# balaji1312/cassnat_asr_public

Measured on AMD Instinct MI355X. Metric: utterances_per_sec, higher is better.
Workload: dtype bf16; 1 GPU; BASELINE configs[1]: CASS-NAT 12L-enc / 1+3+2 dec blocks, d_model 256, 4 heads, d_ff 2048, V 5000, greedy NAST; 32 utterances x 1000 frames x 80 fbank per GPU per step; batch_per_gpu=32, frames=1000, feat_dim=80, global_batch=32, parallelism=utterance-sharded x1, decode_pipelines_per_gpu=2, batches_per_engine_pass=10, utterances_per_engine_pass=320, row_predictions=208, row_predictions_missed=0

## Files before the change

cassnat_asr_public_amd/csrc/conv2.hip:

```cpp
#include <algorithm>
#include <cmath>
#include <cstdlib>
#include <cstring>

#include "kernels.h"

struct Conv2Params {
    const unsigned char* A;
    const unsigned char* W;
    const unsigned char* A_lo;
    const unsigned char* W_lo;
    const int* q8;
    const unsigned char* A8l;
    const unsigned char* A8q;
    const unsigned char* W8q;
    const unsigned char* W8l;
    float out8_scale;
    const float* bias;
    bf16* out;
    int M, T1, F1, T2, F2, ntiles;
    long long lda_bytes;
    int ksteps;
    float* out_f32;
    const float* pe;
    int pe_period;
    float scale;
};

constexpr int C2_BM = 256, C2_N = 256, C2_C = 256, C2_ROWB = 128;
constexpr int C2_SLAB = C2_BM * C2_ROWB;
constexpr int C2_WBASE = 3 * C2_SLAB;
constexpr int C2_OSTRIDE = 528;
constexpr int C2_LDS = 5 * C2_SLAB;
static_assert(C2_BM * C2_OSTRIDE <= C2_LDS && C2_BM == C2_N, "epilogue image fits; A and W slabs are the same size");
static_assert(C2_LDS <= 160 * 1024, "LDS budget");
constexpr int C2_KSTEPS = 9 * (C2_C / 64);
constexpr int C2_LIN8_KSTEPS = 40;

#define C2_STR2(x) #x
#define C2_STR(x) C2_STR2(x)
#define C2_MF CN_MFMA16_ASM
#define C2_DMA(src, dst)                                                                              \
    __builtin_amdgcn_global_load_lds((const __attribute__((address_space(1))) void*)(src),          \
                                     (__attribute__((address_space(3))) void*)(dst), 16, 0, 0)
#ifdef C2_EXP_NO_READ
#define C2_RDA(i) ""
#define C2_RDW(i) ""
#else
#define C2_RDA(i) "ds_read_b128 %[na" #i "], %[an] offset:" C2_STR(i * 4096) "\n\t"
// ... 43 lines not shown
#define C2_BLOCK8(PRE, A0c, W0c, A1c, W1c, A0n, W0n, A1n, W1n, DMA, vo)                                        \
    asm volatile(PRE "s_waitcnt lgkmcnt(0)\n\t"                                                                \
                 C2_M8(0, 0) C2_RDA8(0) C2_M8(0, 1) C2_RDA8(1) C2_M8(0, 2) C2_RDA8(2) C2_M8(0, 3) C2_RDA8(3)   \
                 C2_M8(1, 0) C2_RDW8(0) C2_M8(1, 1) C2_RDW8(1) C2_M8(1, 2) C2_RDW8(2) C2_M8(1, 3) C2_RDW8(3)   \
                 C2_M8(2, 0) DMA(0) C2_M8(2, 1) DMA(1) C2_M8(2, 2) DMA(2) C2_M8(2, 3) DMA(3)                   \
                 C2_M8(3, 0) DMA(4) C2_M8(3, 1) DMA(5) C2_M8(3, 2) DMA(6) C2_M8(3, 3) DMA(7)                   \
                 : [c00] "+a"(acc[0]), [c01] "+a"(acc[1]), [c02] "+a"(acc[2]), [c03] "+a"(acc[3]), [c10] "+a"(acc[4]), \
                   [c11] "+a"(acc[5]), [c12] "+a"(acc[6]), [c13] "+a"(acc[7]), [c20] "+a"(acc[8]), [c21] "+a"(acc[9]), \
                   [c22] "+a"(acc[10]), [c23] "+a"(acc[11]), [c30] "+a"(acc[12]), [c31] "+a"(acc[13]),          \
                   [c32] "+a"(acc[14]), [c33] "+a"(acc[15]), [na0] "=&v"(A0n[0]), [na1] "=&v"(A0n[1]),          \
                   [na2] "=&v"(A0n[2]), [na3] "=&v"(A0n[3]), [nb0] "=&v"(A1n[0]), [nb1] "=&v"(A1n[1]),          \
                   [nb2] "=&v"(A1n[2]), [nb3] "=&v"(A1n[3]), [nw0] "=&v"(W0n[0]), [nw1] "=&v"(W0n[1]),          \
                   [nw2] "=&v"(W0n[2]), [nw3] "=&v"(W0n[3]), [nv0] "=&v"(W1n[0]), [nv1] "=&v"(W1n[1]),          \
                   [nv2] "=&v"(W1n[2]), [nv3] "=&v"(W1n[3]), [tv] "+v"(tv_)                                    \
                 : [a0] "v"(C2_JOIN(A0c[0], A1c[0])), [a1] "v"(C2_JOIN(A0c[1], A1c[1])), [a2] "v"(C2_JOIN(A0c[2], A1c[2])), \
                   [a3] "v"(C2_JOIN(A0c[3], A1c[3])), [w0] "v"(C2_JOIN(W0c[0], W1c[0])), [w1] "v"(C2_JOIN(W0c[1], W1c[1])), \
                   [w2] "v"(C2_JOIN(W0c[2], W1c[2])), [w3] "v"(C2_JOIN(W0c[3], W1c[3])), [an0] "v"(an0_), [an1] "v"(an1_), \
                   [wn0] "v"(wn0_), [wn1] "v"(wn1_), [vo0] "v"(vo[0]), [vo1] "v"(vo[1]), [vo2] "v"(vo[2]), [vo3] "v"(vo[3]), \
                   [vo4] "v"(vo[4]), [vo5] "v"(vo[5]), [vo6] "v"(vo[6]), [vo7] "v"(vo[7]), [st] "s"(st_), [sb] "s"(sb_), \
                   [qa] "v"(qa_), [qb] "v"(qb_), [wstep] "s"(wstep_)                                           \
                 : "memory", "scc")
typedef int c2_v4i __attribute__((ext_vector_type(4)));

template <bool LINEAR, bool X3 = false, bool F8 = false, bool MIX = false>
__global__ __launch_bounds__(256) void conv2_kernel(Conv2Params p) {
    static_assert(!(LINEAR && X3) && !(F8 && X3), "the split form exists for the convolution only; e4m3: convolution and linear_out");
    static_assert(!MIX || (!LINEAR && !X3 && !F8), "MIX is a form of the convolution of its own");
    constexpr int ES = F8 ? 1 : 2;
    extern __shared__ __attribute__((aligned(16))) unsigned char smem[];
    const int tid = threadIdx.x, lane = tid & 63;
    const int wave = __builtin_amdgcn_readfirstlane(tid >> 6);
    const int wm = wave >> 1, wnn = wave & 1;
    const int half = lane >> 5, l31 = lane & 31;
    const int nwg = gridDim.x, xcd = blockIdx.x & 7, q = nwg >> 3, rm = nwg & 7;
    const int tile = (xcd < rm ? xcd * (q + 1) : rm * (q + 1) + (xcd - rm) * q) + (blockIdx.x >> 3);
    const int m0 = tile * C2_BM;

    const int r8 = lane >> 3, cp = lane & 7;
    const unsigned sw = (unsigned)((cp ^ ((4 * wave + (r8 >> 1)) & 7)) << 4);
    const int F1p = p.F1 + 2;
    auto a_off = [&](int mm, int es) -> long long {
        if constexpr (LINEAR) return (long long)mm * p.lda_bytes;
        const int f2 = mm % p.F2, bt = mm / p.F2;
        const int t2 = bt % p.T2, b = bt / p.T2;
        return (((long long)b * (p.T1 + 2) + 2 * t2) * F1p + 2 * f2) * (C2_C * es);
    };
    long long tile_off = a_off(m0, ES);
    unsigned pa[8], pw[8];
#pragma unroll
    for (int i = 0; i < 8; ++i) {
        const int row = 8 * (wave + 4 * i) + r8;
        const int m = m0 + row;
        const int mc = m < p.M ? m : p.M - 1;
        pa[i] = (unsigned)(a_off(mc, ES) - tile_off) + sw;
        if constexpr (LINEAR)
            pw[i] = (unsigned)(row * (p.ksteps * 128)) + sw;
        else
            pw[i] = (unsigned)(row * (9 * C2_C * ES)) + sw;
// ... 332 lines not shown
            for (int g = 0; g < 4; ++g) bv[g] = *reinterpret_cast<const f32x4*>(p.bias + wnn * 128 + 32 * nt + 8 * g + 4 * half);
#pragma unroll
            for (int mt = 0; mt < 4; ++mt)
#pragma unroll
                for (int g = 0; g < 4; ++g) {
                    bf16x4 o;
#pragma unroll
                    for (int e = 0; e < 4; ++e) o[e] = (bf16)fmaxf(acc[4 * nt + mt][4 * g + e] + bv[g][e], 0.f);
                    *reinterpret_cast<bf16x4*>(orow + mt * 32 * C2_OSTRIDE + (32 * nt + 8 * g) * 2) = o;
                }
        }
    }
    __syncthreads();
#pragma unroll
    for (int it = 0; it < 32; ++it) {
        const int row = 8 * it + (tid >> 5), ch = tid & 31;
        const int m = m0 + row;
        if (m < p.M)
            *reinterpret_cast<uint4*>(reinterpret_cast<unsigned char*>(p.out) + (long long)m * 512 + ch * 16) =
                *reinterpret_cast<const uint4*>(smem + row * C2_OSTRIDE + ch * 16);
    }
}

bool conv2_dma_applies(int prec, int C, int N) { return prec == CN_PREC_BF16 && C == C2_C && N == C2_N && !cn_exp_env("CASSNAT_NO_CONV2_DMA"); }

static bool conv2_tile_span_too_large(int T1, int F1, int F2) {
    const long long span = ((256ll / (F2 > 0 ? F2 : 1) + 3) * 2 + 4) * (F1 + 2) * C2_C * 2;
    if (span >= (1ll << 32)) {
        cn_set_error("conv2: one 256-row tile spans more than 4 GiB of the image (feature dimension too wide for the LDS-DMA kernel)");
        return true;
    }
    (void)T1;
    return false;
}

int launch_conv2_dma(const void* in, const void* w, const float* bias, void* out, int B, int T1, int F1, int T2, int F2,
                     hipStream_t s) {
    static CnAttrOnce attr_once;
    int attr_dev;
    if (attr_once.need(&attr_dev)) {
        CN_HIP_CHECK(hipFuncSetAttribute((const void*)conv2_kernel<false>, hipFuncAttributeMaxDynamicSharedMemorySize, C2_LDS));
        attr_once.mark(attr_dev);
    }
    Conv2Params p;
    p.A = (const unsigned char*)in;
    p.W = (const unsigned char*)w;
// ... 123 lines not shown
    p.A8l = p.A + 2 * cells;
    p.A8q = p.A + 3 * cells;
    p.W = (const unsigned char*)w_hi;
    p.W8q = (const unsigned char*)w8q;
    p.W8l = (const unsigned char*)w8l;
    p.q8 = q8_dev;
    p.bias = bias;
    p.out = (bf16*)out;
    p.M = B * T2 * F2;
    p.T1 = T1;
    p.F1 = F1;
    p.T2 = T2;
    p.F2 = F2;
    p.ntiles = cn_ceil_div(p.M, C2_BM);
    if (p.M <= 0) return 0;
    hipLaunchKernelGGL((conv2_kernel<false, false, false, true>), dim3(p.ntiles), dim3(256), C2_LDS, s, p);
    CN_HIP_CHECK(hipGetLastError());
    return 0;
}

bool linear256_dma_applies(int prec, int N, int K) { return prec == CN_PREC_BF16 && N == C2_N && K % 64 == 0 && K >= 128 && !cn_exp_env("CASSNAT_NO_LINEAR_DMA"); }

int launch_linear256_dma(const void* A, int lda, const void* W, const float* bias, float* out, int M, int K, float scale,
                         const float* pe, int pe_period, hipStream_t s) {
    static CnAttrOnce attr_once;
    int attr_dev;
    if (attr_once.need(&attr_dev)) {
        CN_HIP_CHECK(hipFuncSetAttribute((const void*)conv2_kernel<true>, hipFuncAttributeMaxDynamicSharedMemorySize, C2_LDS));
        attr_once.mark(attr_dev);
    }
    if (M <= 0) return 0;
    if (256ll * lda * 2 >= (1ll << 32)) {
        cn_set_error("linear256: a 256-row tile of A exceeds the 32-bit lane offsets of the LDS-DMA kernel");
        return -1;
    }
    Conv2Params p = {};
    p.A = (const unsigned char*)A;
    p.W = (const unsigned char*)W;
    p.bias = bias;
    p.M = M;
    p.T1 = p.F1 = p.T2 = p.F2 = 1;
    p.ntiles = cn_ceil_div(M, C2_BM);
    p.lda_bytes = (long long)lda * 2;
    p.ksteps = K / 64;
    p.out_f32 = out;
    p.pe = pe;
    p.pe_period = pe_period > 0 ? pe_period : 1;
    p.scale = scale;
    hipLaunchKernelGGL(conv2_kernel<true>, dim3(p.ntiles), dim3(256), C2_LDS, s, p);
    CN_HIP_CHECK(hipGetLastError());
    return 0;
}

template <typename F>
static void c2_each_weight(const float* w, int C, long long s_co, long long s_tap, long long s_ci, F f) {
    size_t e = 0;
    for (int co = 0; co < C; ++co)
        for (int tap = 0; tap < 9; ++tap)
            for (int ci = 0; ci < C; ++ci) f(e++, w[co * s_co + tap * s_tap + ci * s_ci]);
}
static int c2_e4m3_exp(const float* w, int C, long long s_co, long long s_tap, long long s_ci) {
    float mx = 0.f;
    c2_each_weight(w, C, s_co, s_tap, s_ci, [&](size_t, float v) { mx = std::max(mx, std::fabs(v)); });
    return cn_e4m3_exp(mx);
}

int pack_conv2_f8(const float* w, int C, long long s_co, long long s_tap, long long s_ci, unsigned char* out) {
    const int lg = c2_e4m3_exp(w, C, s_co, s_tap, s_ci);
    const float scale = std::ldexp(1.f, lg);
    c2_each_weight(w, C, s_co, s_tap, s_ci, [&](size_t e, float v) { out[e] = cn_f32_to_e4m3_host(v * scale); });
    return lg;
// ... 16 lines not shown
```

cassnat_asr_public_amd/csrc/gemm.hip:

```cpp
#include "kernels.h"

struct GemmParams {
    const unsigned char* A;
    const unsigned char* W;
    const float* bias;
    void* C;
    const float* resid;
    const float* pe;
    long long lda_bytes;
    int ldc, ldr;
    int M, N, K;
    int epi;
    int pe_period;
    float scale, resid_scale;
    const float* w_inv_scale;
    float acc_scale, c_scale;
    int ntn;
    int cT1, cF1, cC, cT2, cF2;
};

template <typename T, typename TC, int BM, int BN, bool CONV, bool FULLK = false>
__global__ __launch_bounds__(256) void gemm_kernel(GemmParams p) {
    constexpr int ROWB = 128;
    constexpr int BK = ROWB / (int)sizeof(T);
// ... 280 lines not shown

static int dispatch_gemm_fp8(const GemmArgs& a, hipStream_t s) {
    if (a.M <= 0 || a.N <= 0) return 0;
    if (a.conv || a.K <= 0 || a.K % 128 != 0 || a.lda % 16 != 0) {
        cn_set_error("gemm(fp8): K must be a positive multiple of 128 and rows 16-byte aligned; no convolution form");
        return -1;
    }
    const bool use_big = (long long)cn_ceil_div(a.M, 128) * cn_ceil_div(a.N, 128) >= 512;
    if (a.c_f32) return use_big ? run_gemm<fp8_t, float, 128, 128, false>(a, s) : run_gemm<fp8_t, float, 64, 64, false>(a, s);
    if (a.c_fp8) return use_big ? run_gemm<fp8_t, fp8_t, 128, 128, false>(a, s) : run_gemm<fp8_t, fp8_t, 64, 64, false>(a, s);
    return use_big ? run_gemm<fp8_t, bf16, 128, 128, false>(a, s) : run_gemm<fp8_t, bf16, 64, 64, false>(a, s);
}

int launch_gemm(int prec, const GemmArgs& a, hipStream_t s) {
    if (a.ab_fp8) return dispatch_gemm_fp8(a, s);
    if (a.conv && a.conv_halo) {
        if (!(a.epi == CN_EPI_RELU && a.ldc == a.N && conv2_dma_applies(prec, a.cC, a.N))) {
            cn_set_error("gemm: a haloed conv input is only understood by the bf16 256-channel conv2 kernel");
            return -1;
        }
        return launch_conv2_dma(a.A, a.W, a.bias, a.C, a.cB, a.cT1, a.cF1, a.cT2, a.cF2, s);
    }
    if (!a.conv && a.epi == CN_EPI_EMBED && a.c_f32 && a.ldc == a.N && a.K >= 1024 && linear256_dma_applies(prec, a.N, a.K))
        return launch_linear256_dma(a.A, a.lda, a.W, a.bias, (float*)a.C, a.M, a.K, a.scale, a.pe, a.pe_period, s);
    if (prec == CN_PREC_X3) {
        if (a.lda % 32 != 0 || (!a.c_f32 && a.ldc % 32 != 0)) {
            cn_set_error("gemm: split-bf16 operands need row strides that are multiples of 32 elements");
            return -1;
        }
        return dispatch_gemm<split_t>(a, s);
    }
    return prec == CN_PREC_F32 ? dispatch_gemm<float>(a, s) : dispatch_gemm<bf16>(a, s);
}
```

cassnat_asr_public_amd/csrc/kernels.h:

```cpp
#pragma once
#include "common.h"

enum { CN_PREC_F32 = 0, CN_PREC_BF16 = 1, CN_PREC_X3 = 3 };
static inline size_t cn_elem_size(int prec) { return prec == CN_PREC_BF16 ? 2 : 4; }

enum { CN_EPI_RELU = 1, CN_EPI_RESID = 2, CN_EPI_EMBED = 4, CN_EPI_SWISH = 8 };
struct GemmArgs {
    const void* A = nullptr;
    int lda = 0;
    const void* W = nullptr;
    const float* bias = nullptr;
    void* C = nullptr;
    int ldc = 0;
    int c_f32 = 0;
    int M = 0, N = 0, K = 0;
    int epi = 0;
    const float* resid = nullptr;
    float resid_scale = 1.0f;
    int ldr = 0;
    const float* pe = nullptr;
    int pe_period = 1;
    float scale = 1.f;
    int ab_fp8 = 0;
    float acc_scale = 1.f;
    const float* w_inv_scale = nullptr;
    int c_fp8 = 0;
    float c_scale = 1.f;
    int conv = 0;
    int conv_halo = 0;
    int cB = 0, cT1 = 0, cF1 = 0, cC = 0, cT2 = 0, cF2 = 0;
};
int launch_gemm(int prec, const GemmArgs& a, hipStream_t s);

struct UttMeta {
    int frames;
    int tp;
    int sub_lo;
    int sub_hi;
};
int launch_conv1(int prec, const float* x, const float* w9c, const float* bias, void* out, int B, int T, int F, int T1,
                 int F1, int C, int halo, hipStream_t s, const UttMeta* utt_meta = nullptr);
int launch_conv1_planes(const float* x, const float* w9c, const float* bias, void* out, int B, int T, int F, int T1, int F1,
                        int C, int halo, hipStream_t s, const UttMeta* utt_meta = nullptr);
int launch_conv1_mixplanes(const float* x, const float* w9c, const float* bias, void* out, int B, int T, int F, int T1, int F1, int C,
                           int halo, float scale_l, float scale_q, hipStream_t s, const UttMeta* utt_meta = nullptr);
int launch_conv1_f8(const float* x, const float* w9c, const float* bias, void* out8, int B, int T, int F, int T1, int F1, int C,
                    int halo, float scale, hipStream_t s, const UttMeta* utt_meta = nullptr);
bool conv1_bordered_bf16_applies(int C, int F1);
int launch_conv1_bordered_bf16(const float* x, const float* w9c, const float* bias, void* out, int B, int T, int F, int T1, int F1,
                               int C, hipStream_t s, const UttMeta* utt_meta = nullptr);
constexpr int CN_MAX_SUB = 64;
struct SubList {
    int n;
// ... 190 lines not shown
                   long long capacity);
int launch_wave_resample(int in_rate, int out_rate, const unsigned char* staged, long long staged_bytes, const int* off, const int* samples,
                         const int* channels, const int* channel, int utts, const int* rows, int n_rows, long long max_out, float* out,
                         const int* out_off, hipStream_t s);

bool conv2_dma_applies(int prec, int C, int N);
bool conv2_f8_applies(int C, int N);
int launch_conv2_f8(const void* in8, const void* w8, const int* q8_dev, const float* bias, void* out, int B, int T1, int F1, int T2,
                    int F2, hipStream_t s, float out8_scale = 0.f);
bool linear256_f8_applies(int N, int K);
int launch_linear256_f8(const void* A8, const void* W8, const int* q8_dev, const float* bias, float* out, int M, int K, float scale,
                        const float* pe, int pe_period, hipStream_t s);
bool conv2_mix_applies(int prec, int C, int N);
int launch_conv2_mix(const void* img, const void* w_hi, const void* w8q, const void* w8l, const int* q8_dev, const float* bias, void* out,
                     int B, int T1, int F1, int T2, int F2, hipStream_t s);
constexpr int MIX_LG_AQ = 0, MIX_LG_AL = 11;
int pack_conv2_f8(const float* w, int C, long long s_co, long long s_tap, long long s_ci, unsigned char* out);
void pack_conv2_mix(const float* w, int C, long long s_co, long long s_tap, long long s_ci, unsigned char* out, int* q8);
bool conv2_x3_applies(int prec, int C, int N);
int launch_conv2_x3(const void* in_hi, const void* in_lo, const void* w_hi, const void* w_lo, const float* bias, void* out, int B,
                    int T1, int F1, int T2, int F2, hipStream_t s);
bool linear256_dma_applies(int prec, int N, int K);
int launch_linear256_dma(const void* A, int lda, const void* W, const float* bias, float* out, int M, int K, float scale,
                         const float* pe, int pe_period, hipStream_t s);
int launch_conv2_dma(const void* in, const void* w, const float* bias, void* out, int B, int T1, int F1, int T2, int F2,
                     hipStream_t s);

constexpr int CHAIN_TAB_FLOATS = 5120;
constexpr int CHAIN_UNIT_BYTES = 16384;
struct ChainArgs {
    float* x = nullptr;
    const void* ctx = nullptr;
    int ldctx = 0;
    int ctx_blocked = 0;
    const void* wstream = nullptr;
    const float* tab = nullptr;
    void* out = nullptr;
    int ldo = 0;
    void* ln_out = nullptr;
    int ld_ln = 0;
    int M = 0, d = 0, dff = 0, tail_n = 0, has_next = 0;
    const int* m_dev = nullptr;
    int x_in_blocked = 0, x_out_blocked = 0, store_x = 1;
    int out_blocked = 0;
    int swish = 0;
    int f8 = 0;
    const int* f8_q = nullptr;
// ... 199 lines not shown
```

cassnat_asr_public_amd/csrc/model.hip:

```cpp
#include <algorithm>
#include <cmath>
#include <cstring>
#include <map>
#include <memory>
#include <string>
#include <thread>
#include <vector>

#include "../../include/cassnat_hip.h"
#include "kernels.h"

static thread_local std::string g_last_error;
static const int g_lib_tag = 0;
void cn_set_error(const std::string& msg) { g_last_error = msg; }
extern "C" const char* cn_last_error(void) { return g_last_error.c_str(); }
extern "C" const char* cn_version(void) { return "cassnat_hip 0.1 (gfx950, 16-bit operand " CN_OP16_NAME ")"; }
extern "C" const char* cn_operand16(void) { return CN_OP16_NAME; }

int cn_own_precision(int32_t precision, const char* who) {
#ifdef CN_OP16_F16
    if (precision == CN_PRECISION_F16) return CN_PREC_BF16;
    cn_set_error(std::string(who) + ": this build of the library (libcassnat_hip_f16.so) holds the fp16 engine only (CN_PRECISION_F16)");
    return -1;
#else
// ... 1858 lines not shown
        if (mix_planes) {
            const size_t wn = (size_t)d * 9 * d;
            const unsigned char* w = (const unsigned char*)m->conv2_mixw;
            CN_TRY(launch_conv2_mix(m->c1, w, w + 2 * wn, w + 3 * wn, m->conv2_mixq, m->conv2.b, m->c2, B, T1, F1, Tp, F2, s));
        } else if (x3_planes) {
            const size_t img = (size_t)B * (T1 + 2) * (F1 + 2) * d * 2, wpl = (size_t)d * 9 * d * 2;
            CN_TRY(launch_conv2_x3(m->c1, (const unsigned char*)m->c1 + img, m->conv2_x3w, (const unsigned char*)m->conv2_x3w + wpl,
                                   m->conv2.b, m->c2, B, T1, F1, Tp, F2, s));
        } else if (f8_img) {
            CN_TRY(launch_conv2_f8(m->c1, m->conv2_f8w, m->conv2_f8q, m->conv2.b, m->c2, B, T1, F1, Tp, F2, s, f8_lin ? FP8_S_IMG : 0.f));
        } else {
            CN_TRY(launch_gemm(m->prec, g, s));
        }
    }
    if (cap && !f8_lin) CN_TRY(capture(m, "conv2", m->c2, true, CN_DTYPE_F32, {B, Tp, F2, d}, s));
    if (f8_lin) {
        ProfScope ps(m, "linear_out_embed", 2.0 * M * d * (double)F2 * d, (double)M * F2 * d + (double)d * F2 * d + (double)M * d * 4, s);
        CN_TRY(launch_linear256_f8(m->c2, m->linear_f8w, m->linear_f8q, m->linear_out.b, m->x, M, F2 * d, sqrtf((float)d),
                                   c.conf_enc ? nullptr : m->pe, Tp, s));
    } else {
        GemmArgs g;
        g.A = m->c2;
        g.lda = F2 * d;
        g.W = m->linear_out.W;
        g.bias = m->linear_out.b;
        g.C = m->x;
        g.ldc = d;
        g.c_f32 = 1;
        g.M = M;
        g.N = d;
        g.K = F2 * d;
        g.epi = CN_EPI_EMBED;
        g.pe = c.conf_enc ? nullptr : m->pe;
        g.pe_period = Tp;
        g.scale = sqrtf((float)d);
        ProfScope ps(m, "linear_out_embed", 2.0 * g.M * g.N * g.K,
                     ((double)g.M * g.K + (double)g.N * g.K) * m->es + (double)g.M * g.N * 4, s);
        CN_TRY(launch_gemm(m->prec, g, s));
    }
    if (cap) CN_TRY(capture(m, "x_embed", m->x, false, CN_DTYPE_F32, {B, Tp, d}, s));
    static const bool no_chain_c = cn_exp_env("CASSNAT_NO_CHAIN") != nullptr;
    if (c.conf_enc && !m->enc.empty() && m->enc[0].cf_a.w && !no_chain_c) {
        for (size_t n = 0; n < m->enc.size(); ++n) {
            const bool last = n + 1 == m->enc.size();
            const int xin = (cap || n == 0) ? 0 : CHX_IN_BLK, xout = cap ? 0 : (last ? CHX_NO_STORE : CHX_OUT_BLK);
            CN_TRY(run_conformer_layer_chain(m, m->enc[n], m->x, B, Tp, m->keymask, nullptr, false, 0, nullptr, cap, xin, xout,
                                             last ? m->enc_h : nullptr, s));
            if (cap) CN_TRY(capture(m, ("enc_layer" + std::to_string(n)).c_str(), m->x, false, CN_DTYPE_F32, {B, Tp, d}, s));
        }
        if (cap) CN_TRY(capture(m, "enc_h", m->enc_h, true, CN_DTYPE_F32, {B, Tp, d}, s));
        return 0;
    }
    if (c.conf_enc) {
        for (size_t n = 0; n < m->enc.size(); ++n) {
            CN_TRY(run_conformer_self_layer(m, m->enc[n], m->x, B, Tp, m->keymask, nullptr, s));
            if (cap) CN_TRY(capture(m, ("enc_layer" + std::to_string(n)).c_str(), m->x, false, CN_DTYPE_F32, {B, Tp, d}, s));
        }
        CN_TRY(run_ln(m, m->enc_norm, m->x, m->enc_h, M, s));
        if (cap) CN_TRY(capture(m, "enc_h", m->enc_h, true, CN_DTYPE_F32, {B, Tp, d}, s));
        return 0;
    }
    static const bool no_chain = cn_exp_env("CASSNAT_NO_CHAIN") != nullptr;
    if (m->fp8_enc && (m->enc_chain.size() != m->enc.size() || no_chain)) {
// ... 1899 lines not shown
```

cassnat_asr_public_amd/csrc/ops.hip:

```cpp
#include <algorithm>
#include <cmath>
#include <cstring>
#include <string>
#include <thread>
#include <vector>

#include "../../include/cassnat_hip.h"
#include "kernels.h"

namespace {

class Scratch {
  public:
    Scratch(const char* who, hipStream_t s) : who_(who), s_(s) {}
    Scratch(const Scratch&) = delete;
    Scratch& operator=(const Scratch&) = delete;
    ~Scratch() {
        (void)hipStreamSynchronize(s_);
        for (void* p : bufs_) (void)hipFree(p);
    }
    bool ok() const { return ok_; }
    void* alloc(size_t bytes) {
        if (!ok_) return nullptr;
        void* p = nullptr;
// ... 306 lines not shown
    g.N = C;
    g.K = 9 * C;
    g.epi = CN_EPI_RELU;
    g.conv = 1;
    g.cB = B;
    g.cT1 = T1;
    g.cF1 = F1;
    g.cC = C;
    g.cT2 = T2;
    g.cF2 = F2;
    if (!conv2_dma_applies(precision, C, C)) return launch_gemm(precision, g, (hipStream_t)stream);
    const size_t cell = (size_t)C * 2, prow = (size_t)(F1 + 2) * cell;
    Scratch sc("cn_op_conv2", (hipStream_t)stream);
    void* padded = sc.alloc((size_t)B * (T1 + 2) * prow);
    if (!sc.ok()) return -2;
    CN_HIP_CHECK(hipMemsetAsync(padded, 0, (size_t)B * (T1 + 2) * prow, (hipStream_t)stream));
    for (int b = 0; b < B; ++b)
        CN_HIP_CHECK(hipMemcpy2DAsync((unsigned char*)padded + ((size_t)b * (T1 + 2) + 1) * prow + cell, prow,
                                      (const unsigned char*)conv1_out + (size_t)b * T1 * F1 * cell, (size_t)F1 * cell,
                                      (size_t)F1 * cell, T1, hipMemcpyDeviceToDevice, (hipStream_t)stream));
    g.A = padded;
    g.conv_halo = 1;
    return sc.finish(launch_gemm(precision, g, (hipStream_t)stream));
}

extern "C" int cn_op_layernorm(int32_t precision, const float* x, const float* a2, const float* b2, void* y, int32_t M,
                               int32_t d, float eps, void* stream) {
    if ((precision = cn_own_precision(precision, "cn_op_layernorm")) < 0) return -1;
    return launch_layernorm(precision, x, a2, b2, y, 0, M, d, eps, (hipStream_t)stream);
}

static int conv_module_dims(const char* who, int precision, long long rows, long long row_len, int d, const char* what) {
    if (precision != CN_PREC_F32 && precision != CN_PREC_BF16 && precision != CN_PREC_X3) {
        cn_set_error(std::string(who) + ": precision must be F32, BF16 (F16 in the half-precision build) or BF16X3");
        return -1;
    }
    if (precision == CN_PREC_X3 && d % 32 != 0) {
        cn_set_error(std::string(who) + ": split-bf16 (bf16x3) rows are groups of 32 elements: d % 32 != 0 has no layout");
        return -1;
    }
    if (row_len * d > 0x7fffffffLL || rows * row_len > 0x7fffffffLL || rows * row_len * d >= (1LL << 39)) {
        cn_set_error(std::string(who) + ": " + what + " exceeds the kernels' int arithmetic (2^31 - 1; all elements together: 2^39)");
        return -1;
    }
    return 0;
}
// ... 1033 lines not shown
```

cassnat_asr_public_amd/hip.py:

```python
import ctypes as C
import os
import re

import numpy as np

_HERE = os.path.dirname(os.path.abspath(__file__))
LIB_PATH = os.environ.get("CASSNAT_HIP_LIB") or os.path.join(_HERE, "libcassnat_hip.so")
LIB_PATH_F16 = os.path.join(_HERE, "libcassnat_hip_f16.so")
HEADER_PATH = os.path.join(os.path.dirname(_HERE), "include", "cassnat_hip.h")

PRECISION = {"fp32": 0, "f32": 0, "float32": 0, "bf16": 1, "bfloat16": 1, "fp8": 2, "bf16x3": 3, "fp16": 4, "float16": 4}
DTYPES = {0: np.float32, 1: np.int32, 2: np.uint8, 3: np.float64}
FP8_SCOPE_BITS = {"conv2": 1, "linear": 2, "ffn": 4}


def parse_fp8_scope(text):
    text = (text or "all").strip().lower()
    if text == "all":
        return 0, 0
    scope, first = 0, 0
    for part in text.split("+"):
        name, _, arg = part.strip().partition(":")
        if name not in FP8_SCOPE_BITS or (arg and name != "ffn"):
            raise ValueError(f"hip_fp8_scope: unknown part {part!r} (all, or conv2 / linear / ffn[:first layer] joined by +)")
# ... 71 lines not shown
def lib(flavour=None):
    path = LIB_PATH_F16 if flavour == "f16" else LIB_PATH
    if path in _libs:
        return _libs[path]
    if not os.path.exists(path):
        raise HipError(f"{path} is missing: run `python -c 'import __graft_entry__ as g; g.build()'` "
                       "(there is no CPU fallback for the CASS-NAT hot path)")
    L = C.CDLL(path)
    L.cn_last_error.restype = C.c_char_p
    L.cn_version.restype = C.c_char_p
    L.cn_operand16.restype = C.c_char_p
    L.cn_model_destroy.restype = None
    for name in declared_symbols():
        fn = getattr(L, name)
        if name not in ("cn_last_error", "cn_version", "cn_operand16", "cn_model_destroy"):
            fn.restype = C.c_int
    L.cn_op_gemm.argtypes = [C.c_int32, C.c_void_p, C.c_int32, C.c_void_p, C.c_void_p, C.c_void_p, C.c_int32, C.c_int32,
                             C.c_int32, C.c_int32, C.c_int32, C.c_int32, C.c_void_p, C.c_int32, C.c_void_p, C.c_int32,
                             C.c_float, C.c_void_p]
    L.cn_op_convert.argtypes = [C.c_int32, C.c_void_p, C.c_void_p, C.c_int64, C.c_int32, C.c_void_p]
    L.cn_op_conv1.argtypes = [C.c_int32] + [C.c_void_p] * 4 + [C.c_int32] * 4 + [C.c_void_p]
    L.cn_op_conv1_bordered.argtypes = [C.c_void_p] * 4 + [C.c_int32] * 4 + [C.c_void_p]
    L.cn_op_conv2.argtypes = [C.c_int32] + [C.c_void_p] * 4 + [C.c_int32] * 4 + [C.c_void_p]
    L.cn_op_conv_frontend_fp8.argtypes = [C.c_void_p] * 7 + [C.c_int32] * 4 + [C.c_float, C.c_float, C.c_void_p, C.c_void_p]
    L.cn_op_conv_frontend_mix.argtypes = [C.c_void_p] * 7 + [C.c_int32] * 4 + [C.c_void_p]
    L.cn_op_linear256_fp8.argtypes = [C.c_void_p] * 4 + [C.c_int32] * 2 + [C.c_float, C.c_float, C.c_void_p, C.c_int32, C.c_void_p, C.c_void_p]
    L.cn_op_layernorm.argtypes = [C.c_int32] + [C.c_void_p] * 4 + [C.c_int32, C.c_int32, C.c_float, C.c_void_p]
    L.cn_op_glu.argtypes = [C.c_int32, C.c_void_p, C.c_void_p, C.c_int32, C.c_int32, C.c_void_p]
    L.cn_op_dwconv.argtypes = [C.c_int32] + [C.c_void_p] * 4 + [C.c_int32] * 5 + [C.c_void_p]
    L.cn_op_groupnorm_swish.argtypes = [C.c_int32] + [C.c_void_p] * 5 + [C.c_int32] * 3 + [C.c_float, C.c_void_p]
    L.cn_op_attention.argtypes = [C.c_int32, C.c_void_p, C.c_int32, C.c_void_p, C.c_int32, C.c_void_p, C.c_int32,
                                  C.c_void_p, C.c_int32, C.c_int32, C.c_int32, C.c_int32, C.c_int32, C.c_void_p,
                                  C.c_void_p, C.c_void_p, C.c_int32, C.c_int32, C.c_float, C.c_void_p]
    L.cn_op_attention_desc.argtypes = [C.c_int32, C.POINTER(CnAttnDesc), C.c_void_p]
    L.cn_attn_desc_size.argtypes = []
    L.cn_op_attention_packed.argtypes = [C.c_int32, C.POINTER(CnAttnDesc), C.c_void_p, C.c_int32, C.c_void_p]
    L.cn_op_row_plan.argtypes = [C.c_void_p, C.c_int32, C.c_int32, C.c_int32, C.c_int32, C.c_void_p, C.c_void_p, C.c_void_p, C.c_void_p]
    L.cn_op_logsoftmax_argmax.argtypes = [C.c_void_p, C.c_int32, C.c_int32, C.c_void_p, C.c_void_p, C.c_int32, C.c_void_p]
    L.cn_op_ctc_align.argtypes = [C.c_void_p] * 3 + [C.c_int32] * 5 + [C.c_void_p] * 6
    L.cn_op_greedy_pack.argtypes = [C.c_void_p] * 3 + [C.c_int32] * 4 + [C.c_void_p] * 4
    L.cn_op_ctc_prefix_beam.argtypes = [C.c_void_p, C.c_void_p, C.c_int32, C.c_int32, C.c_int32, C.c_int32, C.c_int32, C.c_double,
                                        C.c_int32, C.c_void_p, C.c_int32, C.c_void_p, C.c_void_p, C.c_void_p, C.c_void_p, C.c_void_p,
                                        C.c_void_p]
    L.cn_op_ctc_viterbi.argtypes = [C.c_void_p] * 5 + [C.c_int32] * 6 + [C.c_void_p, C.c_void_p]
    L.cn_op_topk.argtypes = [C.c_void_p, C.c_int32, C.c_int32, C.c_int32, C.c_void_p, C.c_void_p, C.c_void_p]
    L.cn_op_gemm_fp8.argtypes = [C.c_void_p, C.c_int32, C.c_void_p, C.c_void_p, C.c_void_p, C.c_int32, C.c_int32, C.c_int32, C.c_float,
# ... 289 lines not shown
            self._chk(self.L.cn_model_load_weights(self.handle, name.encode(), a.ctypes.data_as(C.c_void_p), shape, a.ndim),
                  f"load {name}")
        pe = np.ascontiguousarray(pe_table.detach().cpu().numpy() if hasattr(pe_table, "detach") else pe_table,
                                  dtype=np.float32)
        self._chk(self.L.cn_model_load_pe(self.handle, pe.ctypes.data_as(C.c_void_p), pe.shape[0]), "load pe")
        self.finalize()

    def finalize(self):
        self._chk(self.L.cn_model_finalize(self.handle), "cn_model_finalize")
        self.finalized = True

    def weight_blob(self):
        p, n = C.c_void_p(), C.c_int64()
        self._chk(self.L.cn_model_weight_blob(self.handle, C.byref(p), C.byref(n)), "cn_model_weight_blob")
        return p.value, n.value

    @staticmethod
    def make_opts(args, capture=False):
        opts = CnDecodeOpts(padding_idx=int(args.padding_idx), sos=1, left_trigger=int(getattr(args, "left_trigger", 0)),
                            right_trigger=int(getattr(args, "right_trigger", 0)), src_trigger=int(bool(getattr(args, "src_trigger", False))),
                            use_unimask=int(bool(getattr(args, "use_unimask", False))), beam_width=int(args.beam_width),
                            capture=int(bool(capture)), no_trigger=int(not getattr(args, "use_trigger", True)))
        opts.reserved[1] = int(bool(getattr(args, "hip_padded_rows", False)))
        return opts

    def decode(self, feats, size_ratio, opts, hyp, hyp_len, score):
        B, T, F = feats.shape
        self._chk(self.L.cn_decode_nast(self.handle, _ptr(feats), _ptr(size_ratio), B, T, F, C.byref(opts), _ptr(hyp),
                                    hyp.shape[1], _ptr(hyp_len), _ptr(score), current_stream()), "cn_decode_nast")

    def decode_merged(self, feats, size_ratio, opts, sub_rows, sub_frames, hyp, hyp_len, score, u_hint=0):
        B, T, F = feats.shape
        n = len(sub_rows) if sub_rows is not None else 0
        rows = (C.c_int32 * max(1, n))(*[int(x) for x in (sub_rows or [])])
        frames = (C.c_int32 * max(1, n))(*[int(x) for x in (sub_frames or [])])
        ticket = C.c_int32(-1)
        self._chk(self.L.cn_decode_nast_merged(self.handle, _ptr(feats), _ptr(size_ratio), B, T, F, C.byref(opts), n, rows, frames,
                                           int(u_hint), _ptr(hyp), hyp.shape[1], _ptr(hyp_len), _ptr(score), current_stream(),
                                           C.byref(ticket)), "cn_decode_nast_merged")
        return ticket.value

    def check_range(self, what="decode"):
        if self.precision not in ("fp16", "float16", "bf16x3"):
            return
        fault, limit = C.c_int32(), C.c_float()
        self._chk(self.L.cn_take_range_fault(self.handle, C.byref(fault), C.byref(limit)), "cn_take_range_fault")
# ... 173 lines not shown
```

include/cassnat_hip.h:

```cpp
#ifndef CASSNAT_HIP_H
#define CASSNAT_HIP_H
#include <stdint.h>

#ifdef __cplusplus
extern "C" {
#endif

typedef struct cn_model cn_model;

enum { CN_PRECISION_F32 = 0, CN_PRECISION_BF16 = 1, CN_PRECISION_FP8 = 2, CN_PRECISION_BF16X3 = 3, CN_PRECISION_F16 = 4 };
enum { CN_DTYPE_F32 = 0, CN_DTYPE_I32 = 1, CN_DTYPE_U8 = 2, CN_DTYPE_F64 = 3 };

typedef struct cn_config {
    int32_t input_size;
    int32_t d_model, n_head, d_encff, d_decff;
    int32_t n_enc, n_extra, n_self_dec, n_mix_dec;
    int32_t vocab_size;
    int32_t precision;
    int32_t max_batch;
    int32_t max_frames;
    int32_t device;
    int32_t ast;
    int32_t conf_enc, conf_dec;
    int32_t enc_max_rel, dec_max_rel;
// ... 156 lines not shown
                        const int32_t* samples_dev, const int32_t* channels_dev, const int32_t* channel_dev,
                        const int32_t* channels_host, const int32_t* channel_host, int32_t utts, const int32_t* rows_dev,
                        int32_t rows, int64_t max_out, float* wave_dev, const int32_t* out_off_dev, void* stream);

int cn_op_convert(int32_t precision, const void* src, void* dst, int64_t n, int32_t to_f32, void* stream);
int cn_op_gemm(int32_t precision, const void* A, int32_t lda, const void* W, const float* bias, void* C, int32_t ldc,
               int32_t c_is_f32, int32_t M, int32_t N, int32_t K, int32_t relu, const float* resid, int32_t ldr,
               const float* pe, int32_t pe_period, float scale, void* stream);
int cn_op_conv1(int32_t precision, const float* x, const float* w9c, const float* bias, void* out, int32_t B, int32_t T,
                int32_t F, int32_t C, void* stream);
int cn_op_conv1_bordered(const float* x, const float* w9c, const float* bias, void* out, int32_t B, int32_t T, int32_t F,
                         int32_t C, void* stream);
int cn_op_conv_frontend_fp8(const float* x_dev, const float* w1_9c_dev, const float* b1_dev, const float* w2_host,
                            const float* b2_dev, void* out_dev, void* img8_out_dev, int32_t B, int32_t T, int32_t F, int32_t C,
                            float img_scale, float out8_scale, float* w_scale_out, void* stream);

int cn_op_conv_frontend_mix(const float* x, const float* w1_9c, const float* b1, const float* w2_host, const float* b2, void* out,
                            void* img_out , int32_t B, int32_t T, int32_t F,
                            int32_t C, void* stream);
int cn_op_linear256_fp8(const void* a8_dev, const float* w_host, const float* bias_dev, float* out_dev, int32_t M, int32_t K,
                        float a_scale, float out_scale, const float* pe_dev, int32_t pe_period, float* w_scale_out, void* stream);
int cn_op_conv2(int32_t precision, const void* conv1_out, const void* w_khwc, const float* bias, void* out, int32_t B,
                int32_t T1, int32_t F1, int32_t C, void* stream);
int cn_op_layernorm(int32_t precision, const float* x, const float* a2, const float* b2, void* y, int32_t M, int32_t d,
                    float eps, void* stream);
int cn_op_glu(int32_t precision, const void* in, void* out, int32_t M, int32_t d, void* stream);
int cn_op_dwconv(int32_t precision, const void* x, const float* w, const float* bias, float* y, int32_t B, int32_t L, int32_t d,
                 int32_t k, int32_t form, void* stream);
int cn_op_groupnorm_swish(int32_t precision, const float* x, double* stats, const float* gw, const float* gb, void* out, int32_t B,
                          int32_t L, int32_t d, float eps, void* stream);
int cn_op_attention(int32_t precision, const void* Q, int32_t ldq, const void* K, int32_t ldk, const void* V,
                    int32_t ldv, void* O, int32_t ldo, int32_t B, int32_t H, int32_t Lq, int32_t Lk,
                    const uint8_t* keymask, const int32_t* klen, const int32_t* intervals, int32_t iv_stride,
                    int32_t causal, float scale, void* stream);
typedef struct cn_attn_desc {
    const void* Q;
    const void* K;
    const void* V;
    void* O;
    int32_t ldq, ldk, ldv, ldo;
    int32_t B, H, Lq, Lk;
    const uint8_t* keymask;
    int32_t kv_mod;
    const int32_t* kv_index;
    const int32_t* klen;
    const int32_t* kcap;
// ... 143 lines not shown
```

Baseline: 51800 utt/s.

## Balance linear_out tail wave with 128-row tiles in a mixed-tile kernel

The linear_out embedding GEMM now launches a mixed kernel. It runs as many 256-row tiles as fill whole waves of CUs, then covers the remaining rows with smaller 128-row tiles using a new 4-stage A / 3-stage W LDS-DMA pipeline. The aim is to cut tail-wave imbalance when the 256-row tile count is not a multiple of the CU count. The new 128-row path carries extra code and register pressure, and its per-tile efficiency may be lower. A host option keeps the old all-256 path, and a public op exposes both forms.

```diff
diff --git a/cassnat_asr_public_amd/csrc/conv2.hip b/cassnat_asr_public_amd/csrc/conv2.hip
--- a/cassnat_asr_public_amd/csrc/conv2.hip
+++ b/cassnat_asr_public_amd/csrc/conv2.hip
@@ -25,6 +25,7 @@
     const float* pe;
     int pe_period;
     float scale;
+    int n256;
 };
 
 constexpr int C2_BM = 256, C2_N = 256, C2_C = 256, C2_ROWB = 128;
@@ -114,8 +115,13 @@
                  : "memory", "scc")
 typedef int c2_v4i __attribute__((ext_vector_type(4)));
 
-template <bool LINEAR, bool X3 = false, bool F8 = false, bool MIX = false>
-__global__ __launch_bounds__(256) void conv2_kernel(Conv2Params p) {
+__device__ __forceinline__ int c2_xcd_tile(int wg, int nwg) {
+    const int xcd = wg & 7, q = nwg >> 3, rm = nwg & 7;
+    return (xcd < rm ? xcd * (q + 1) : rm * (q + 1) + (xcd - rm) * q) + (wg >> 3);
+}
+
+template <bool LINEAR, bool X3, bool F8, bool MIX>
+__device__ __forceinline__ void conv2_tile(const Conv2Params p, const int tile) {
     static_assert(!(LINEAR && X3) && !(F8 && X3), "the split form exists for the convolution only; e4m3: convolution and linear_out");
     static_assert(!MIX || (!LINEAR && !X3 && !F8), "MIX is a form of the convolution of its own");
     constexpr int ES = F8 ? 1 : 2;
@@ -124,8 +130,6 @@
     const int wave = __builtin_amdgcn_readfirstlane(tid >> 6);
     const int wm = wave >> 1, wnn = wave & 1;
     const int half = lane >> 5, l31 = lane & 31;
-    const int nwg = gridDim.x, xcd = blockIdx.x & 7, q = nwg >> 3, rm = nwg & 7;
-    const int tile = (xcd < rm ? xcd * (q + 1) : rm * (q + 1) + (xcd - rm) * q) + (blockIdx.x >> 3);
     const int m0 = tile * C2_BM;
 
     const int r8 = lane >> 3, cp = lane & 7;
@@ -504,6 +508,169 @@
     }
 }
 
+template <bool LINEAR, bool X3 = false, bool F8 = false, bool MIX = false>
+__global__ __launch_bounds__(256) void conv2_kernel(Conv2Params p) {
+    conv2_tile<LINEAR, X3, F8, MIX>(p, c2_xcd_tile(blockIdx.x, gridDim.x));
+}
+
+#define L1_DMA_A0 C2_DMA_I(0)
+#define L1_DMA_A1 C2_DMA_I(1)
+#define L1_DMA_A2 C2_DMA_I(2)
+#define L1_DMA_A3 C2_DMA_I(3)
+#define L1_DMA_A4 ""
+#define L1_DMA_A5 ""
+#define L1_DMA_A6 ""
+#define L1_DMA_A7 ""
+#define L1_DMA_A(i) L1_DMA_A##i
+#define L1_BLOCK(PRE, Ac, Wc, An, Wn, DMA, vo)                                                                 \
+    asm volatile(PRE "s_waitcnt lgkmcnt(0)\n\t"                                                                \
+                 C2_M(C2_MF, 0, 0) C2_RDA(0) C2_RDA(1) C2_M(C2_MF, 0, 1) C2_RDW(0) C2_RDW(1)                   \
+                 C2_M(C2_MF, 1, 0) C2_RDW(2) C2_RDW(3) C2_M(C2_MF, 1, 1) DMA(0) DMA(1)                         \
+                 C2_M(C2_MF, 2, 0) DMA(2) DMA(3) C2_M(C2_MF, 2, 1) DMA(4) DMA(5)                               \
+                 C2_M(C2_MF, 3, 0) DMA(6) DMA(7) C2_M(C2_MF, 3, 1)                                             \
+                 : [c00] "+a"(acc[0]), [c01] "+a"(acc[1]), [c10] "+a"(acc[2]), [c11] "+a"(acc[3]), [c20] "+a"(acc[4]), \
+                   [c21] "+a"(acc[5]), [c30] "+a"(acc[6]), [c31] "+a"(acc[7]), [na0] "=&v"(An[0]), [na1] "=&v"(An[1]), \
+                   [nw0] "=&v"(Wn[0]), [nw1] "=&v"(Wn[1]), [nw2] "=&v"(Wn[2]), [nw3] "=&v"(Wn[3])              \
+                 : [a0] "v"(Ac[0]), [a1] "v"(Ac[1]), [w0] "v"(Wc[0]), [w1] "v"(Wc[1]), [w2] "v"(Wc[2]), [w3] "v"(Wc[3]), \
+                   [an] "v"(an_), [wn] "v"(wn_), [vo0] "v"(vo[0]), [vo1] "v"(vo[1]), [vo2] "v"(vo[2]), [vo3] "v"(vo[3]), \
+                   [vo4] "v"(vo[4]), [vo5] "v"(vo[5]), [vo6] "v"(vo[6]), [vo7] "v"(vo[7]), [st] "s"(st_), [sb] "s"(sb_) \
+                 : "memory", "scc")
+constexpr int L1_BM = 128;
+constexpr int L1_ASLAB = L1_BM * C2_ROWB;
+constexpr int L1_WBASE = 4 * L1_ASLAB;
+static_assert(L1_WBASE + 3 * C2_SLAB <= C2_LDS, "the 128-row tile's stages fit the launch's LDS");
+
+__device__ __forceinline__ void linear128_tile(const Conv2Params p, const int m0) {
+    extern __shared__ __attribute__((aligned(16))) unsigned char smem[];
+    const int tid = threadIdx.x, lane = tid & 63;
+    const int wave = __builtin_amdgcn_readfirstlane(tid >> 6);
+    const int wm = wave >> 1, wnn = wave & 1;
+    const int half = lane >> 5, l31 = lane & 31;
+    const int r8 = lane >> 3, cp = lane & 7;
+    const unsigned sw = (unsigned)((cp ^ ((4 * wave + (r8 >> 1)) & 7)) << 4);
+    const long long tile_off = (long long)m0 * p.lda_bytes;
+    unsigned pa[8], pw[8];
+#pragma unroll
+    for (int i = 0; i < 8; ++i) {
+        const int row = 8 * (wave + 4 * i) + r8;
+        const int m = m0 + (row & (L1_BM - 1));
+        const int mc = m < p.M ? m : p.M - 1;
+        pa[i] = (unsigned)((long long)(mc - m0) * p.lda_bytes) + sw;
+        pw[i] = (unsigned)(row * (p.ksteps * 128)) + sw;
+    }
+    const unsigned lds0 = (unsigned)(size_t)(__attribute__((address_space(3))) unsigned char*)smem;
+    const unsigned m0_wave = __builtin_amdgcn_readfirstlane(lds0 + wave * 1024);
+    const int KSTEPS = p.ksteps, KL = KSTEPS - 1;
+    auto a_base = [&](int kt) -> const unsigned char* { return p.A + tile_off + (long long)kt * 128; };
+    auto w_base = [&](int kt) -> const unsigned char* { return p.W + (long long)kt * 128; };
+    auto a_dst = [&](int k4) -> unsigned { return m0_wave + (unsigned)(k4 * L1_ASLAB); };
+    auto w_dst = [&](int k3) -> unsigned { return m0_wave + (unsigned)(L1_WBASE + k3 * C2_SLAB); };
+#define L1_ISSUE(n, dst, vo, sbase)                                                                           \
+    {                                                                                                         \
+        const unsigned d_ = (dst);                                                                            \
+        const unsigned char* s_ = (sbase);                                                                    \
+        _Pragma("unroll") for (int i_ = 0; i_ < n; ++i_)                                                      \
+            asm volatile("s_mov_b32 m0, %0\n\ts_nop 0\n\tglobal_load_lds_dwordx4 %1, %2" ::"s"(d_ + i_ * 4096), "v"(vo[i_]), \
+                         "s"(s_) : "memory");                                                                 \
+    }
+    const unsigned off0 = (((unsigned)half) ^ (unsigned)((l31 >> 1) & 7)) << 4;
+    const unsigned a_rd0 = lds0 + (unsigned)((wm * 64 + l31) * C2_ROWB) + off0;
+    const unsigned w_rd0 = lds0 + (unsigned)(L1_WBASE + (wnn * 128 + l31) * C2_ROWB) + off0;
+
+    f32x16 acc[8];
+#pragma unroll
+    for (int i = 0; i < 8; ++i)
+#pragma unroll
+        for (int r = 0; r < 16; ++r) acc[i][r] = 0.f;
+    bf16x8 Ax[2], Wx[4], Ay[2], Wy[4];
+
+#define L1_PRE3 "s_waitcnt lgkmcnt(0)\n\ts_waitcnt vmcnt(16)\n\ts_barrier\n\t"
+    L1_ISSUE(4, a_dst(0), pa, a_base(0))
+    L1_ISSUE(8, w_dst(0), pw, w_base(0))
+    L1_ISSUE(4, a_dst(1), pa, a_base(min(1, KL)))
+    L1_ISSUE(8, w_dst(1), pw, w_base(min(1, KL)))
+    L1_ISSUE(4, a_dst(2), pa, a_base(min(2, KL)))
+    asm volatile("s_waitcnt vmcnt(16)\n\ts_barrier" ::: "memory");
+    {
+        const unsigned an_ = a_rd0, wn_ = w_rd0;
+        asm volatile("ds_read_b128 %0, %6\n\tds_read_b128 %1, %6 offset:4096\n\tds_read_b128 %2, %7\n\t"
+                     "ds_read_b128 %3, %7 offset:4096\n\tds_read_b128 %4, %7 offset:8192\n\tds_read_b128 %5, %7 offset:12288"
+                     : "=&v"(Ax[0]), "=&v"(Ax[1]), "=&v"(Wx[0]), "=&v"(Wx[1]), "=&v"(Wx[2]), "=&v"(Wx[3])
+                     : "v"(an_), "v"(wn_)
+                     : "memory");
+    }
+    int k3 = 0;
+    for (int kt = 0; kt < KSTEPS; ++kt) {
+        const int k3n = k3 == 2 ? 0 : k3 + 1, k3p = k3 == 0 ? 2 : k3 - 1;
+        const unsigned so_a = (unsigned)((kt & 3) * L1_ASLAB), so_w = (unsigned)(k3 * C2_SLAB);
+        const unsigned sn_a = (unsigned)(((kt + 1) & 3) * L1_ASLAB), sn_w = (unsigned)(k3n * C2_SLAB);
+        {
+            const unsigned an_ = C2_RD(a_rd0, 1, so_a), wn_ = C2_RD(w_rd0, 1, so_w);
+            const unsigned* vo = pw;
+            const unsigned st_ = w_dst(k3p);
+            const unsigned char* sb_ = w_base(min(kt + 2, KL));
+            L1_BLOCK("", Ax, Wx, Ay, Wy, C2_DMA_I, vo);
+        }
+        {
+            const unsigned an_ = C2_RD(a_rd0, 2, so_a), wn_ = C2_RD(w_rd0, 2, so_w);
+            const unsigned* vo = pa;
+            const unsigned st_ = a_dst((kt + 3) & 3);
+            const unsigned char* sb_ = a_base(min(kt + 3, KL));
+            L1_BLOCK("", Ay, Wy, Ax, Wx, L1_DMA_A, vo);
+        }
+        {
+            const unsigned an_ = C2_RD(a_rd0, 3, so_a), wn_ = C2_RD(w_rd0, 3, so_w);
+            const unsigned st_ = 0;
+            const unsigned char* sb_ = p.W;
+            const unsigned* vo = pw;
+            L1_BLOCK("", Ax, Wx, Ay, Wy, C2_NODMA, vo);
+        }
+        {
+            const unsigned an_ = a_rd0 + sn_a, wn_ = w_rd0 + sn_w;
+            const unsigned st_ = 0;
+            const unsigned char* sb_ = p.W;
+            const unsigned* vo = pw;
+            L1_BLOCK(L1_PRE3, Ay, Wy, Ax, Wx, C2_NODMA, vo);
+        }
+        k3 = k3n;
+    }
+    asm volatile("s_nop 13\n\ts_waitcnt lgkmcnt(0)\n\ts_waitcnt vmcnt(0)"
+                 : "+v"(Ax[0]), "+v"(Ax[1]), "+v"(Wx[0]), "+v"(Wx[1]), "+v"(Wx[2]), "+v"(Wx[3]), "+v"(Ay[0]), "+v"(Ay[1]), "+v"(Wy[0]),
+                   "+v"(Wy[1]), "+v"(Wy[2]), "+v"(Wy[3])
+                 :: "memory");
+#pragma unroll
+    for (int mt = 0; mt < 2; ++mt) {
+        const int mrow = m0 + wm * 64 + 32 * mt + l31;
+        if (mrow >= p.M) continue;
+        float* orow = p.out_f32 + (long long)mrow * C2_N + wnn * 128 + 4 * half;
+        const float* prow = p.pe ? p.pe + (long long)(mrow % p.pe_period) * C2_N + wnn * 128 + 4 * half : nullptr;
+#pragma unroll
+        for (int nt = 0; nt < 4; ++nt)
+#pragma unroll
+            for (int g = 0; g < 4; ++g) {
+                const f32x4 bv = *reinterpret_cast<const f32x4*>(p.bias + wnn * 128 + 32 * nt + 8 * g + 4 * half);
+                f32x4 o;
+#pragma unroll
+                for (int e = 0; e < 4; ++e) o[e] = (acc[2 * nt + mt][4 * g + e] + bv[e]) * p.scale;
+                if (prow) {
+                    const f32x4 pv = *reinterpret_cast<const f32x4*>(prow + 32 * nt + 8 * g);
+#pragma unroll
+                    for (int e = 0; e < 4; ++e) o[e] += pv[e];
+                }
+                *reinterpret_cast<f32x4*>(orow + 32 * nt + 8 * g) = o;
+            }
+        asm volatile("" ::: "memory");
+    }
+}
+
+__global__ __launch_bounds__(256) void conv2_linear_mixed_kernel(Conv2Params p) {
+    const int wg = blockIdx.x;
+    if (wg < p.n256)
+        conv2_tile<true, false, false, false>(p, c2_xcd_tile(wg, p.n256));
+    else
+        linear128_tile(p, p.n256 * C2_BM + c2_xcd_tile(wg - p.n256, (int)gridDim.x - p.n256) * L1_BM);
+}
+
 bool conv2_dma_applies(int prec, int C, int N) { return prec == CN_PREC_BF16 && C == C2_C && N == C2_N && !cn_exp_env("CASSNAT_NO_CONV2_DMA"); }
 
 static bool conv2_tile_span_too_large(int T1, int F1, int F2) {
@@ -673,13 +840,19 @@
 bool linear256_dma_applies(int prec, int N, int K) { return prec == CN_PREC_BF16 && N == C2_N && K % 64 == 0 && K >= 128 && !cn_exp_env("CASSNAT_NO_LINEAR_DMA"); }
 
 int launch_linear256_dma(const void* A, int lda, const void* W, const float* bias, float* out, int M, int K, float scale,
-                         const float* pe, int pe_period, hipStream_t s) {
+                         const float* pe, int pe_period, hipStream_t s, int cus) {
     static CnAttrOnce attr_once;
+    static std::atomic<int> dev_cus[64];
     int attr_dev;
     if (attr_once.need(&attr_dev)) {
         CN_HIP_CHECK(hipFuncSetAttribute((const void*)conv2_kernel<true>, hipFuncAttributeMaxDynamicSharedMemorySize, C2_LDS));
+        CN_HIP_CHECK(hipFuncSetAttribute((const void*)conv2_linear_mixed_kernel, hipFuncAttributeMaxDynamicSharedMemorySize, C2_LDS));
+        int n = 0;
+        CN_HIP_CHECK(hipDeviceGetAttribute(&n, hipDeviceAttributeMultiprocessorCount, attr_dev));
+        dev_cus[attr_dev].store(n > 0 ? n : 1);
         attr_once.mark(attr_dev);
     }
+    if (cus == 0) cus = dev_cus[attr_dev].load();
     if (M <= 0) return 0;
     if (256ll * lda * 2 >= (1ll << 32)) {
         cn_set_error("linear256: a 256-row tile of A exceeds the 32-bit lane offsets of the LDS-DMA kernel");
@@ -698,6 +871,13 @@
     p.pe = pe;
     p.pe_period = pe_period > 0 ? pe_period : 1;
     p.scale = scale;
+    if (cus > 0) {
+        p.n256 = p.ntiles / cus * cus;
+        const int n128 = cn_ceil_div(M - std::min(M, p.n256 * C2_BM), L1_BM);
+        hipLaunchKernelGGL(conv2_linear_mixed_kernel, dim3(p.n256 + n128), dim3(256), C2_LDS, s, p);
+        CN_HIP_CHECK(hipGetLastError());
+        return 0;
+    }
     hipLaunchKernelGGL(conv2_kernel<true>, dim3(p.ntiles), dim3(256), C2_LDS, s, p);
     CN_HIP_CHECK(hipGetLastError());
     return 0;
diff --git a/cassnat_asr_public_amd/csrc/gemm.hip b/cassnat_asr_public_amd/csrc/gemm.hip
--- a/cassnat_asr_public_amd/csrc/gemm.hip
+++ b/cassnat_asr_public_amd/csrc/gemm.hip
@@ -326,7 +326,7 @@
         return launch_conv2_dma(a.A, a.W, a.bias, a.C, a.cB, a.cT1, a.cF1, a.cT2, a.cF2, s);
     }
     if (!a.conv && a.epi == CN_EPI_EMBED && a.c_f32 && a.ldc == a.N && a.K >= 1024 && linear256_dma_applies(prec, a.N, a.K))
-        return launch_linear256_dma(a.A, a.lda, a.W, a.bias, (float*)a.C, a.M, a.K, a.scale, a.pe, a.pe_period, s);
+        return launch_linear256_dma(a.A, a.lda, a.W, a.bias, (float*)a.C, a.M, a.K, a.scale, a.pe, a.pe_period, s, a.lin_cus);
     if (prec == CN_PREC_X3) {
         if (a.lda % 32 != 0 || (!a.c_f32 && a.ldc % 32 != 0)) {
             cn_set_error("gemm: split-bf16 operands need row strides that are multiples of 32 elements");
diff --git a/cassnat_asr_public_amd/csrc/kernels.h b/cassnat_asr_public_amd/csrc/kernels.h
--- a/cassnat_asr_public_amd/csrc/kernels.h
+++ b/cassnat_asr_public_amd/csrc/kernels.h
@@ -29,6 +29,7 @@
     int conv = 0;
     int conv_halo = 0;
     int cB = 0, cT1 = 0, cF1 = 0, cC = 0, cT2 = 0, cF2 = 0;
+    int lin_cus = 0;
 };
 int launch_gemm(int prec, const GemmArgs& a, hipStream_t s);
 
@@ -265,7 +266,7 @@
                     int T1, int F1, int T2, int F2, hipStream_t s);
 bool linear256_dma_applies(int prec, int N, int K);
 int launch_linear256_dma(const void* A, int lda, const void* W, const float* bias, float* out, int M, int K, float scale,
-                         const float* pe, int pe_period, hipStream_t s);
+                         const float* pe, int pe_period, hipStream_t s, int cus = 0);
 int launch_conv2_dma(const void* in, const void* w, const float* bias, void* out, int B, int T1, int F1, int T2, int F2,
                      hipStream_t s);
 
diff --git a/cassnat_asr_public_amd/csrc/model.hip b/cassnat_asr_public_amd/csrc/model.hip
--- a/cassnat_asr_public_amd/csrc/model.hip
+++ b/cassnat_asr_public_amd/csrc/model.hip
@@ -1904,6 +1904,7 @@
         GemmArgs g;
         g.A = m->c2;
         g.lda = F2 * d;
+        g.lin_cus = (o->reserved[2] & 1) ? -1 : 0;
         g.W = m->linear_out.W;
         g.bias = m->linear_out.b;
         g.C = m->x;
@@ -1920,7 +1921,7 @@
                      ((double)g.M * g.K + (double)g.N * g.K) * m->es + (double)g.M * g.N * 4, s);
         CN_TRY(launch_gemm(m->prec, g, s));
     }
-    if (cap) CN_TRY(capture(m, "x_embed", m->x, false, CN_DTYPE_F32, {B, Tp, d}, s));
+    if (cap || (o->reserved[2] & 2)) CN_TRY(capture(m, "x_embed", m->x, false, CN_DTYPE_F32, {B, Tp, d}, s));
     static const bool no_chain_c = cn_exp_env("CASSNAT_NO_CHAIN") != nullptr;
     if (c.conf_enc && !m->enc.empty() && m->enc[0].cf_a.w && !no_chain_c) {
         for (size_t n = 0; n < m->enc.size(); ++n) {
diff --git a/cassnat_asr_public_amd/csrc/ops.hip b/cassnat_asr_public_amd/csrc/ops.hip
--- a/cassnat_asr_public_amd/csrc/ops.hip
+++ b/cassnat_asr_public_amd/csrc/ops.hip
@@ -352,6 +352,21 @@
     g.A = padded;
     g.conv_halo = 1;
     return sc.finish(launch_gemm(precision, g, (hipStream_t)stream));
+}
+
+extern "C" int cn_op_linear256(const void* A, int32_t lda, const void* W, const float* bias, float* out, int32_t M, int32_t K,
+                               float scale, const float* pe, int32_t pe_period, int32_t form, int32_t cus, void* stream) {
+    if (!A || !W || !bias || !out || M < 1 || lda < K || (pe && pe_period < 1) ||
+        (form != CN_LINEAR256_TILES_256 && form != CN_LINEAR256_TILES_BALANCED) || (form == CN_LINEAR256_TILES_BALANCED && cus < 0)) {
+        cn_set_error("cn_op_linear256: bad argument (form: CN_LINEAR256_TILES_256 or CN_LINEAR256_TILES_BALANCED with cus >= 0)");
+        return -1;
+    }
+    if (!linear256_dma_applies(CN_PREC_BF16, 256, K)) {
+        cn_set_error("cn_op_linear256: K must be a multiple of 64, at least 128 (and the LDS-DMA kernel not switched off)");
+        return -1;
+    }
+    return launch_linear256_dma(A, lda, W, bias, out, M, K, scale, pe, pe_period, (hipStream_t)stream,
+                                form == CN_LINEAR256_TILES_256 ? -1 : cus);
 }
 
 extern "C" int cn_op_layernorm(int32_t precision, const float* x, const float* a2, const float* b2, void* y, int32_t M,
diff --git a/cassnat_asr_public_amd/hip.py b/cassnat_asr_public_amd/hip.py
--- a/cassnat_asr_public_amd/hip.py
+++ b/cassnat_asr_public_amd/hip.py
@@ -117,6 +117,8 @@
     L.cn_op_conv1.argtypes = [C.c_int32] + [C.c_void_p] * 4 + [C.c_int32] * 4 + [C.c_void_p]
     L.cn_op_conv1_bordered.argtypes = [C.c_void_p] * 4 + [C.c_int32] * 4 + [C.c_void_p]
     L.cn_op_conv2.argtypes = [C.c_int32] + [C.c_void_p] * 4 + [C.c_int32] * 4 + [C.c_void_p]
+    L.cn_op_linear256.argtypes = [C.c_void_p, C.c_int32] + [C.c_void_p] * 3 + [C.c_int32] * 2 + [C.c_float, C.c_void_p] + \
+                                 [C.c_int32] * 3 + [C.c_void_p]
     L.cn_op_conv_frontend_fp8.argtypes = [C.c_void_p] * 7 + [C.c_int32] * 4 + [C.c_float, C.c_float, C.c_void_p, C.c_void_p]
     L.cn_op_conv_frontend_mix.argtypes = [C.c_void_p] * 7 + [C.c_int32] * 4 + [C.c_void_p]
     L.cn_op_linear256_fp8.argtypes = [C.c_void_p] * 4 + [C.c_int32] * 2 + [C.c_float, C.c_float, C.c_void_p, C.c_int32, C.c_void_p, C.c_void_p]
@@ -452,6 +454,7 @@
                             use_unimask=int(bool(getattr(args, "use_unimask", False))), beam_width=int(args.beam_width),
                             capture=int(bool(capture)), no_trigger=int(not getattr(args, "use_trigger", True)))
         opts.reserved[1] = int(bool(getattr(args, "hip_padded_rows", False)))
+        opts.reserved[2] = int(bool(getattr(args, "hip_linear_out_256", False))) | 2 * int(bool(getattr(args, "hip_keep_x_embed", False)))
         return opts
 
     def decode(self, feats, size_ratio, opts, hyp, hyp_len, score):
diff --git a/include/cassnat_hip.h b/include/cassnat_hip.h
--- a/include/cassnat_hip.h
+++ b/include/cassnat_hip.h
@@ -202,6 +202,10 @@
                         float a_scale, float out_scale, const float* pe_dev, int32_t pe_period, float* w_scale_out, void* stream);
 int cn_op_conv2(int32_t precision, const void* conv1_out, const void* w_khwc, const float* bias, void* out, int32_t B,
                 int32_t T1, int32_t F1, int32_t C, void* stream);
+#define CN_LINEAR256_TILES_256 0
+#define CN_LINEAR256_TILES_BALANCED 1
+int cn_op_linear256(const void* A, int32_t lda, const void* W, const float* bias, float* out, int32_t M, int32_t K, float scale,
+                    const float* pe, int32_t pe_period, int32_t form, int32_t cus, void* stream);
 int cn_op_layernorm(int32_t precision, const float* x, const float* a2, const float* b2, void* y, int32_t M, int32_t d,
                     float eps, void* stream);
 int cn_op_glu(int32_t precision, const void* in, void* out, int32_t M, int32_t d, void* stream);
```

After: 51750 utt/s. No clear change (-0.1%).
